# sid2364/dna-sequences-pg-extension

Hardware: NVIDIA B200
Metric: Gkmer/s counted (k=31) at 1/2/4/8 B200; extraction HBM GB/s vs peak (higher is better)
Workload: dtype u64

## Files before the change

dna-sequences-pg-extension_b200/csrc/dnagpu.cu:

```cuda
#include "../../include/dnagpu.h"

#include <cuda_runtime.h>

#include <algorithm>
#include <cmath>
#include <cstdarg>
#include <cstdio>
#include <cstdlib>
#include <cstring>
#include <new>
#include <string>
#include <thread>
#include <unordered_set>
#include <vector>

#include "kernels.cuh"
#include "partition.cuh"
#include "index.cuh"

using namespace dnagpu;

struct ProfRec {
    std::string name;
    cudaEvent_t e0, e1;
};

struct dnagpu_ctx {
    int device = 0;
    int sm_count = 0;
    cudaStream_t stream = nullptr;
    bool own_stream = true;
    unsigned long long *d_ctr = nullptr;
    int bins_ctas_per_sm = 4;
    unsigned long long *h_ctr = nullptr;
    cudaStream_t copy_stream = nullptr;
    std::vector<dnagpu_ctx *> peers;
    std::vector<uint64_t *> shard_buf;
    std::vector<uint64_t> shard_cap;
    bool profiling = false;
    bool plane_filter = false;
    bool force_exact = false;
    std::vector<ProfRec> prof;
    std::unordered_set<dnagpu_seq *> seqs;
    std::unordered_set<dnagpu_table *> tables;
    std::unordered_set<dnagpu_index *> indexes;
    char err[512] = {0};
};

struct dnagpu_seq {
    dnagpu_ctx *ctx = nullptr;
    int layout = kSingle;
    uint64_t *d_words = nullptr;
    bool own_words = true;
    uint64_t n_words_alloc = 0;
    uint64_t n_words = 0;
    uint64_t n_seqs = 1;
    uint64_t bases = 0;
    uint64_t stride = 0;
    uint64_t start_limit = 0;
    std::vector<uint64_t> h_n_bases;
    uint64_t *d_word_off = nullptr, *d_n_bases = nullptr;
    std::vector<const uint64_t *> piece_ptr;
    std::vector<uint64_t> piece_first, piece_starts;
    int cached_k = 0;
    uint64_t *d_row_off = nullptr, *d_item_off = nullptr;
    uint64_t cached_rows = 0, cached_items = 0;
};

struct dnagpu_table {
    dnagpu_ctx *ctx = nullptr;
    int k = 0;
    uint64_t rows = 0;
    uint64_t *d_kmers = nullptr, *d_counts = nullptr;
    std::vector<dnagpu_table *> parts;
};

struct dnagpu_index {
    dnagpu_ctx *ctx = nullptr;
    int k = 0;
    uint64_t rows = 0;
    uint64_t *d_skeys = nullptr, *d_rows = nullptr;
};

static thread_local char g_err[512] = "";

#ifdef DNAGPU_TUNING
// ... 160 lines not shown
    SMEM_ATTR(k_filter_collect<kSingle>);
    SMEM_ATTR(k_filter_collect<kFixed>);
    SMEM_ATTR(k_filter_collect<kRagged>);
    SMEM_ATTR((k_filter_sa<kSingle, kSaCollect>));
    SMEM_ATTR((k_filter_sa<kFixed, kSaCollect>));
    SMEM_ATTR((k_filter_sa<kSingle, kSaWrite>));
    SMEM_ATTR((k_filter_sa<kFixed, kSaWrite>));
    SMEM_ATTR((k_partition_write<kSingle, false>));
    SMEM_ATTR((k_partition_write<kSingle, true>));
    SMEM_ATTR((k_partition_write<kFixed, false>));
    SMEM_ATTR((k_partition_write<kFixed, true>));
    SMEM_ATTR((k_partition_write<kRagged, false>));
    SMEM_ATTR((k_partition_write<kRagged, true>));
    SMEM_ATTR((k_count_dense_smem<kSingle, false, uint32_t>));
    SMEM_ATTR((k_count_dense_smem<kSingle, true, uint32_t>));
    SMEM_ATTR((k_count_dense_smem<kFixed, false, uint32_t>));
    SMEM_ATTR((k_count_dense_smem<kFixed, true, uint32_t>));
    SMEM_ATTR((k_count_dense_smem<kRagged, false, uint32_t>));
    SMEM_ATTR((k_count_dense_smem<kRagged, true, uint32_t>));
    SMEM_ATTR((k_count_dense_smem<kSingle, false, unsigned long long>));
    SMEM_ATTR((k_count_dense_smem<kSingle, true, unsigned long long>));
    SMEM_ATTR((k_count_dense_smem<kFixed, false, unsigned long long>));
    SMEM_ATTR((k_count_dense_smem<kFixed, true, unsigned long long>));
    SMEM_ATTR((k_count_dense_smem<kRagged, false, unsigned long long>));
    SMEM_ATTR((k_count_dense_smem<kRagged, true, unsigned long long>));
#undef SMEM_ATTR
    {
        const int psmem = kTileKeys * (int)sizeof(uint64_t) + (int)sizeof(ScatterSmem);
#define PSMEM_ATTR(kern) cudaFuncSetAttribute(kern, cudaFuncAttributeMaxDynamicSharedMemorySize, psmem)
        PSMEM_ATTR((k_part_scatter_seq<kSingle, false>));
        PSMEM_ATTR((k_part_scatter_seq<kSingle, true>));
        PSMEM_ATTR((k_part_scatter_seq<kFixed, false>));
        PSMEM_ATTR((k_part_scatter_seq<kFixed, true>));
        PSMEM_ATTR((k_part_scatter_seq<kRagged, false>));
        PSMEM_ATTR((k_part_scatter_seq<kRagged, true>));
        PSMEM_ATTR(k_part_scatter_keys<false>);
        {
            const int psmem32 = 32 * kScatThreads * (int)sizeof(uint64_t) + (int)sizeof(ScatterSmem);
#define PSMEM32_ATTR(kern) cudaFuncSetAttribute(kern, cudaFuncAttributeMaxDynamicSharedMemorySize, psmem32)
            PSMEM32_ATTR((k_part_scatter_keys<false, kBigPerKeys, kBigThreadsKeys>));
            PSMEM32_ATTR((k_part_scatter_keys<true, kBigPerKeys, kBigThreadsKeys>));
            PSMEM32_ATTR((k_part_scatter_seq<kSingle, false, kBigPer, kBigThreads>));
            PSMEM32_ATTR((k_part_scatter_seq<kSingle, true, kBigPer, kBigThreads>));
            PSMEM32_ATTR((k_part_scatter_seq<kFixed, false, kBigPer, kBigThreads>));
            PSMEM32_ATTR((k_part_scatter_seq<kFixed, true, kBigPer, kBigThreads>));
            PSMEM32_ATTR((k_part_scatter_seq<kRagged, false, kBigPer, kBigThreads>));
            PSMEM32_ATTR((k_part_scatter_seq<kRagged, true, kBigPer, kBigThreads>));
#undef PSMEM32_ATTR
        }
        PSMEM_ATTR(k_part_scatter_keys<true>);
#undef PSMEM_ATTR
        {
            int per_sm = 0;
            if (cudaOccupancyMaxActiveBlocksPerMultiprocessor(&per_sm, k_count_buckets_bins, kThreads, 0) == cudaSuccess &&
                per_sm > 0)
                ctx->bins_ctas_per_sm = per_sm;
        }
        cudaFuncSetAttribute(k_sort_scatter<true>, cudaFuncAttributeMaxDynamicSharedMemorySize, (int)sizeof(SortSmem));
        cudaFuncSetAttribute(k_sort_scatter<false>, cudaFuncAttributeMaxDynamicSharedMemorySize, (int)sizeof(SortSmem));
        const int bsmem = kBucketSlots * 12;
        cudaFuncSetAttribute(k_count_buckets<false>, cudaFuncAttributeMaxDynamicSharedMemorySize, bsmem);
        cudaFuncSetAttribute(k_count_buckets<true>, cudaFuncAttributeMaxDynamicSharedMemorySize, bsmem);
    }
    CU(nullptr, cudaGetLastError());
    *out = ctx;
    return DNAGPU_OK;
}

extern "C" int dnagpu_create_multi(dnagpu_ctx **out, const int *devices, int n_devices)
{
    if (!out || !devices || n_devices < 1 || n_devices > kMaxPieces)
        return fail(nullptr, DNAGPU_EARG, "dnagpu_create_multi: need 1..%d devices", kMaxPieces);
    *out = nullptr;
    for (int a = 0; a < n_devices; ++a)
        for (int b = a + 1; b < n_devices; ++b)
            if (devices[a] == devices[b]) return fail(nullptr, DNAGPU_EARG, "device %d is listed twice", devices[a]);
    dnagpu_ctx *ctx = nullptr;
    TRY(dnagpu_create(&ctx, devices[0]));
    for (int d = 1; d < n_devices; ++d) {
        dnagpu_ctx *p = nullptr;
        int rc = dnagpu_create(&p, devices[d]);
        if (rc != DNAGPU_OK) {
            dnagpu_destroy(ctx);
            return rc;
        }
        ctx->peers.push_back(p);
    }
    for (int a = 0; a < n_devices; ++a) {
        cudaSetDevice(devices[a]);
        for (int b = 0; b < n_devices; ++b) {
            if (a == b) continue;
            int can = 0;
            cudaDeviceCanAccessPeer(&can, devices[a], devices[b]);
            cudaError_t e = can ? cudaDeviceEnablePeerAccess(devices[b], 0) : cudaErrorPeerAccessUnsupported;
            if (e == cudaErrorPeerAccessAlreadyEnabled) {
                cudaGetLastError();
                e = cudaSuccess;
            }
            if (e != cudaSuccess) {
                cudaGetLastError();
                dnagpu_destroy(ctx);
                return fail(nullptr, DNAGPU_ENODEVICE, "GPU %d cannot map the memory of GPU %d (%s): no multi-GPU context",
                            devices[a], devices[b], cudaGetErrorString(e));
            }
        }
    }
    cudaSetDevice(devices[0]);
    ctx->shard_buf.assign((size_t)n_devices, nullptr);
    ctx->shard_cap.assign((size_t)n_devices, 0);
// ... 1143 lines not shown
                k_part_hist_seq<LY, true><<<hgrid, kThreads, 0, ctx->stream>>>(in.v, in.p, mask, shift1, P1, hist1);
            else
                k_part_hist_seq<LY, false><<<hgrid, kThreads, 0, ctx->stream>>>(in.v, in.p, mask, shift1, P1, hist1);
        })));
    }
    TRY(scan_any(ctx, sc, (const uint64_t *)hist1, P1, off1));
    uint64_t *out = *keys_io;
    if (in.filtered || out)
        TRY(read_u64(ctx, off1 + P1, &n));
    if (!out) {
        TRY(sc.get((void **)&out, (n + 2) * 8));
        *keys_io = out;
    } else if (cap < n + 2) {
        *n_out = n;
        return fail(ctx, DNAGPU_ECAPACITY, "partition needs room for %llu keys (+2 pad)", (unsigned long long)n);
    }
    if (in.d_keys) {
        TRY(launch(ctx, "part_scatter", [&] {
            k_part_scatter_keys<true><<<grid_for(in.n, kTileKeys), kScatThreads, psmem, ctx->stream>>>(
                in.d_keys, root_off, root_off + 1, root_tiles_scat, 1, 1, shift1, P1, off1, cur1, out, ctx->d_ctr);
        }));
    } else {
        const bool per32 = scatter_tile32(P1, in.d_keys ? 0 : 1);
        if (per32) {
            const int psmem32 = 32 * kScatThreads * (int)sizeof(uint64_t) + (int)sizeof(ScatterSmem);
            const unsigned grid = grid_for(in.v.n_items, kScatThreads);
            DISPATCH_LAYOUT(in.seq->layout, TRY(launch(ctx, "part_scatter", [&] {
                if (in.filtered)
                    k_part_scatter_seq<LY, true, kBigPer, kBigThreads><<<grid, kBigThreads, psmem32, ctx->stream>>>(
                        in.v, in.p, mask, shift1, P1, off1, cur1, out, ctx->d_ctr, 0);
                else
                    k_part_scatter_seq<LY, false, kBigPer, kBigThreads><<<grid, kBigThreads, psmem32, ctx->stream>>>(
                        in.v, in.p, mask, shift1, P1, off1, cur1, out, ctx->d_ctr, 0);
            })));
        } else {
            const unsigned grid = grid_for(in.v.n_items, kScatThreads / 2);
            DISPATCH_LAYOUT(in.seq->layout, TRY(launch(ctx, "part_scatter", [&] {
                if (in.filtered)
                    k_part_scatter_seq<LY, true><<<grid, kScatThreads, psmem, ctx->stream>>>(
                        in.v, in.p, mask, shift1, P1, off1, cur1, out, ctx->d_ctr, 0);
                else
                    k_part_scatter_seq<LY, false><<<grid, kScatThreads, psmem, ctx->stream>>>(
                        in.v, in.p, mask, shift1, P1, off1, cur1, out, ctx->d_ctr, 0);
            })));
        }
    }
    *off1_out = off1;
    *n_out = n;
    return DNAGPU_OK;
}

static int part_finish_impl(dnagpu_ctx *ctx, Scratch &sc, const uint64_t *keys, uint64_t n, const uint64_t *parent_off,
                            const uint64_t *parent_end, uint64_t n_parents, uint64_t n_groups, int b1, int b2, int k,
                            dnagpu_stats *stats, uint64_t total_rows, dnagpu_table **table, bool optimistic2,
                            bool *regions_full)
{
    const int psmem = kTileKeys * (int)sizeof(uint64_t) + (int)sizeof(ScatterSmem);
    const uint64_t *bucket_keys = keys, *bucket_off = parent_off, *bucket_end = parent_end;
    uint64_t n_buckets = n_parents;
    *regions_full = false;
    if (b2 > 0) {
        const uint32_t P2 = 1u << b2;
        const int shift2 = 64 - b1 - b2;
        n_buckets = n_groups * P2;
        unsigned long long *hist2 = nullptr, *cur2;
        uint64_t *off2, *end2 = nullptr, *tiles_hist = nullptr, *tiles_scat, *bufB;
        TileInfo *tparent_hist = nullptr, *tparent_scat = nullptr;
        const uint64_t mean2 = (n + n_buckets - 1) / n_buckets;
        const uint64_t cap2 = mean2 + 7 * (uint64_t)std::ceil(std::sqrt((double)mean2)) + 64;
        TRY(sc.get((void **)&cur2, n_buckets * 8));
        TRY(sc.get((void **)&off2, (n_buckets + 1) * 8));
        CU(ctx, cudaMemsetAsync(cur2, 0, n_buckets * 8, ctx->stream));
        if (optimistic2) {
            TRY(sc.get((void **)&end2, n_buckets * 8));
            TRY(sc.get((void **)&bufB, (n_buckets * cap2 + 2) * 8));
            TRY(launch(ctx, "part_tiles", [&] {
                k_region_begs<<<grid_for(n_buckets, kThreads), kThreads, 0, ctx->stream>>>(cap2, n_buckets, off2);
            }));
        } else {
            TRY(sc.get((void **)&hist2, n_buckets * 8));
            TRY(sc.get((void **)&bufB, (n + 2) * 8));
            CU(ctx, cudaMemsetAsync(hist2, 0, n_buckets * 8, ctx->stream));
            TRY(part_tiles(ctx, sc, parent_off, parent_end, n_parents, kSuperTile, &tiles_hist, &tparent_hist,
                           (uint64_t)grid_for(n, kSuperTile) + n_parents));
        }
        const bool per32 = scatter_tile32(P2, 2);
        TRY(part_tiles(ctx, sc, parent_off, parent_end, n_parents, per32 ? 2 * kTileKeys : kTileKeys, &tiles_scat, &tparent_scat,
                       (uint64_t)grid_for(n, per32 ? 2 * kTileKeys : kTileKeys) + n_parents));
        if (!optimistic2) {
            TRY(launch(ctx, "part_hist2", [&] {
                k_part_hist_keys<<<grid_for(n, kSuperTile) + (unsigned)n_parents, kThreads, 0, ctx->stream>>>(
                    keys, parent_off, parent_end, tiles_hist, n_parents, n_groups, shift2, P2, hist2, tparent_hist);
            }));
            TRY(scan_any(ctx, sc, (const uint64_t *)hist2, n_buckets, off2));
        }
        const uint64_t cap = optimistic2 ? cap2 : 0;
        TRY(launch(ctx, "part_scatter2", [&] {
            if (per32) {
                const int psmem32 = 32 * kScatThreads * (int)sizeof(uint64_t) + (int)sizeof(ScatterSmem);
                k_part_scatter_keys<false, kBigPerKeys, kBigThreadsKeys><<<grid_for(n, 2 * kTileKeys) + (unsigned)n_parents, kBigThreadsKeys, psmem32,
                                                 ctx->stream>>>(keys, parent_off, parent_end, tiles_scat, n_parents, n_groups,
                                                                shift2, P2, off2, cur2, bufB, ctx->d_ctr, cap, C_L2OVF,
                                                                tparent_scat);
            } else {
                k_part_scatter_keys<false><<<grid_for(n, kTileKeys) + (unsigned)n_parents, kScatThreads, psmem, ctx->stream>>>(
                    keys, parent_off, parent_end, tiles_scat, n_parents, n_groups, shift2, P2, off2, cur2, bufB, ctx->d_ctr,
                    cap, C_L2OVF, tparent_scat);
            }
        }));
        bucket_keys = bufB;
        bucket_off = off2;
        bucket_end = off2 + 1;
        if (optimistic2) {
            TRY(launch(ctx, "part_tiles", [&] {
                k_region_ends<<<grid_for(n_buckets, kThreads), kThreads, 0, ctx->stream>>>(cur2, off2, cap2, (uint32_t)n_buckets,
                                                                                         end2);
            }));
            bucket_end = end2;
        }
    }
    const uint64_t spill_cap = std::max<uint64_t>(1ull << 16, n / 64);
    Slot *spill;
    TRY(sc.get((void **)&spill, spill_cap * sizeof(Slot)));
    TRY(launch(ctx, "table_init", [&] {
        k_table_init<<<(unsigned)std::min<uint64_t>(grid_for(spill_cap, kThreads), (uint64_t)ctx->sm_count * 8),
                       kThreads, 0, ctx->stream>>>(spill, spill_cap);
    }));
    const int bsmem = kBucketSlots * 12;
    const unsigned cgrid = (unsigned)std::min<uint64_t>(n_buckets, (uint64_t)ctx->sm_count * (16384 / kBucketSlots));
    static const bool use_bins = !tune_env("DNAGPU_NO_BINS");
    if (use_bins) {
        uint32_t *passed;
        TRY(sc.get((void **)&passed, n_buckets * 4 + 16));
        const unsigned bgrid = (unsigned)std::min<uint64_t>(n_buckets, (uint64_t)ctx->sm_count * ctx->bins_ctas_per_sm);
        TRY(launch(ctx, "count_buckets", [&] {
            k_count_buckets_bins<<<bgrid, kThreads, 0, ctx->stream>>>(bucket_keys, bucket_off, bucket_end, n_buckets,
                                                                     ctx->d_ctr, passed, ctx->d_ctr + C_PASSED);
        }));
        TRY(launch(ctx, "count_buckets_passed", [&] {
            k_count_buckets<false><<<cgrid, kThreads, bsmem, ctx->stream>>>(bucket_keys, bucket_off, bucket_end, n_buckets,
                                                                           spill, spill_cap, ctx->d_ctr, nullptr, nullptr,
                                                                           passed, ctx->d_ctr + C_PASSED);
        }));
    } else {
        TRY(launch(ctx, "count_buckets", [&] {
            k_count_buckets<false><<<cgrid, kThreads, bsmem, ctx->stream>>>(bucket_keys, bucket_off, bucket_end, n_buckets,
                                                                           spill, spill_cap, ctx->d_ctr, nullptr, nullptr);
        }));
    }
    TRY(fetch_counters(ctx));
    if (ctx->h_ctr[C_L2OVF]) {
        *regions_full = true;
        return DNAGPU_OK;
    }
#ifdef DNAGPU_PHASE_TIMING
    fprintf(stderr, "count_buckets phases (cycles/bucket, thread 0): init %.0f | sync %.0f | insert %.0f | prefetch+sync %.0f | buckets %llu\n",
            (double)ctx->h_ctr[110] / ctx->h_ctr[114], (double)ctx->h_ctr[111] / ctx->h_ctr[114],
            (double)ctx->h_ctr[112] / ctx->h_ctr[114], (double)ctx->h_ctr[113] / ctx->h_ctr[114],
            (unsigned long long)ctx->h_ctr[114]);
    fprintf(stderr, "scatter_seq phases (cycles/tile, thread 0): load+rank %.0f | barrier %.0f | plan %.0f | place %.0f+sync | flush %.0f | tiles %llu\n",
            (double)ctx->h_ctr[100] / ctx->h_ctr[105], (double)ctx->h_ctr[101] / ctx->h_ctr[105],
            (double)ctx->h_ctr[102] / ctx->h_ctr[105], (double)ctx->h_ctr[103] / ctx->h_ctr[105],
            (double)ctx->h_ctr[104] / ctx->h_ctr[105], (unsigned long long)ctx->h_ctr[105]);
#endif
    if (ctx->h_ctr[C_OVERFLOW])
        return fail(ctx, DNAGPU_EINTERNAL, "spill table of %llu slots overflowed", (unsigned long long)spill_cap);
    const uint64_t side = ctx->h_ctr[C_SIDE];
    const uint64_t keyed = ctx->h_ctr[C_DISTINCT];
    stats->total = total_rows ? total_rows : ctx->h_ctr[C_TOTAL];
    stats->distinct = keyed + (side > 0);
    stats->unique = ctx->h_ctr[C_UNIQUE] + (side == 1);
    if (table) {
        TRY(table_new(ctx, k, stats->distinct, table));
        if (keyed) {
            CU(ctx, cudaMemsetAsync(ctx->d_ctr + C_CURSOR, 0, 8, ctx->stream));
            TRY(launch(ctx, "count_buckets_emit", [&] {
                k_count_buckets<true><<<cgrid, kThreads, bsmem, ctx->stream>>>(
                    bucket_keys, bucket_off, bucket_end, n_buckets, spill, spill_cap, ctx->d_ctr, (*table)->d_kmers,
                    (*table)->d_counts);
            }));
            TRY(launch(ctx, "table_compact", [&] {
                k_table_compact<<<(unsigned)std::min<uint64_t>(grid_for(spill_cap, kThreads), (uint64_t)ctx->sm_count * 8),
                                  kThreads, 0, ctx->stream>>>(spill, spill_cap, (*table)->d_kmers,
                                                              (*table)->d_counts, ctx->d_ctr);
            }));
        }
        if (side) {
            ctx->h_ctr[0] = kEmpty;
            ctx->h_ctr[1] = side;
            CU(ctx, cudaMemcpyAsync((*table)->d_kmers + keyed, &ctx->h_ctr[0], 8, cudaMemcpyHostToDevice, ctx->stream));
            CU(ctx, cudaMemcpyAsync((*table)->d_counts + keyed, &ctx->h_ctr[1], 8, cudaMemcpyHostToDevice, ctx->stream));
        }
        CU(ctx, cudaStreamSynchronize(ctx->stream));
    }
    return DNAGPU_OK;
}

static int part_finish(dnagpu_ctx *ctx, Scratch &sc, const uint64_t *keys, uint64_t n, const uint64_t *parent_off,
                       const uint64_t *parent_end, uint64_t n_parents, uint64_t n_groups, int b1, int b2, int k,
                       dnagpu_stats *stats, uint64_t total_rows, dnagpu_table **table)
{
    static const bool allow = !tune_env("DNAGPU_EXACT_L2");
    const bool optimistic2 = allow && !ctx->force_exact && b2 > 0 && n_groups == n_parents && (n >> (b1 + b2)) >= 512;
    bool full = false;
    TRY(part_finish_impl(ctx, sc, keys, n, parent_off, parent_end, n_parents, n_groups, b1, b2, k, stats, total_rows, table,
                         optimistic2, &full));
    if (!full) return DNAGPU_OK;
    CU(ctx, cudaMemsetAsync(ctx->d_ctr + C_DISTINCT, 0, 2 * 8, ctx->stream));
    CU(ctx, cudaMemsetAsync(ctx->d_ctr + C_OVERFLOW, 0, 2 * 8, ctx->stream));
    CU(ctx, cudaMemsetAsync(ctx->d_ctr + C_L2OVF, 0, 2 * 8, ctx->stream));
    if (table && *table) {
        dnagpu_table_free(*table);
        *table = nullptr;
    }
    return part_finish_impl(ctx, sc, keys, n, parent_off, parent_end, n_parents, n_groups, b1, b2, k, stats, total_rows, table,
                            false, &full);
}

struct L1Regions {
    uint64_t *keys = nullptr, *beg = nullptr, *end = nullptr;
    unsigned long long *cur = nullptr;
    uint64_t cap = 0;
    uint32_t P1 = 0;
    int b1 = 0;
};

static int l1_regions_begin(dnagpu_ctx *ctx, Scratch &sc, uint64_t n_rows, int b1, L1Regions *r)
{
    r->b1 = b1;
    r->P1 = 1u << b1;
    const uint64_t mean = n_rows >> b1;
    r->cap = mean + mean / 8 + std::min<uint64_t>(65536, std::max<uint64_t>(1024, mean / 2));
    TRY(sc.get((void **)&r->keys, ((uint64_t)r->P1 * r->cap + 2) * 8));
    TRY(sc.get((void **)&r->beg, (uint64_t)r->P1 * 8));
    TRY(sc.get((void **)&r->end, (uint64_t)r->P1 * 8));
    TRY(sc.get((void **)&r->cur, (uint64_t)r->P1 * 8));
    TRY(launch(ctx, "part_tiles", [&] {
        k_region_begs<<<grid_for(r->P1, kThreads), kThreads, 0, ctx->stream>>>(r->cap, r->P1, r->beg);
    }));
    CU(ctx, cudaMemsetAsync(r->cur, 0, (uint64_t)r->P1 * 8, ctx->stream));
    return DNAGPU_OK;
}

static int l1_regions_scatter(dnagpu_ctx *ctx, const L1Regions &r, int layout, const SeqView &v, int k)
{
    const Pred none = {~0ull, ~0ull, ~0ull, ~0ull};
    if (scatter_tile32(r.P1, 1)) {
        const int psmem = 32 * kScatThreads * (int)sizeof(uint64_t) + (int)sizeof(ScatterSmem);
        const unsigned grid = grid_for(v.n_items, kScatThreads);
        DISPATCH_LAYOUT(layout, TRY(launch(ctx, "part_scatter", [&] {
            k_part_scatter_seq<LY, false, kBigPer, kBigThreads><<<grid, kBigThreads, psmem, ctx->stream>>>(
                v, none, kmer_mask(k), 64 - r.b1, r.P1, r.beg, r.cur, r.keys, ctx->d_ctr, r.cap);
        })));
        return DNAGPU_OK;
    }
    const int psmem = kTileKeys * (int)sizeof(uint64_t) + (int)sizeof(ScatterSmem);
    const unsigned grid = grid_for(v.n_items, kScatThreads / 2);
    DISPATCH_LAYOUT(layout, TRY(launch(ctx, "part_scatter", [&] {
        k_part_scatter_seq<LY, false><<<grid, kScatThreads, psmem, ctx->stream>>>(
            v, none, kmer_mask(k), 64 - r.b1, r.P1, r.beg, r.cur, r.keys, ctx->d_ctr, r.cap);
    })));
    return DNAGPU_OK;
}

static int l1_regions_scatter_keys(dnagpu_ctx *ctx, Scratch &sc, const L1Regions &r, const uint64_t *d_keys, uint64_t n)
{
    uint64_t *root_off, *tiles;
    TRY(sc.get((void **)&root_off, 2 * 8));
    ctx->h_ctr[C_COUNT] = 0;
    ctx->h_ctr[C_COUNT + 1] = n;
    CU(ctx, cudaMemcpyAsync(root_off, ctx->h_ctr + C_COUNT, 16, cudaMemcpyHostToDevice, ctx->stream));
    CU(ctx, cudaStreamSynchronize(ctx->stream));
    TRY(part_tiles(ctx, sc, root_off, root_off + 1, 1, 2 * kTileKeys, &tiles));
    const int psmem32 = 32 * kScatThreads * (int)sizeof(uint64_t) + (int)sizeof(ScatterSmem);
    return launch(ctx, "part_scatter", [&] {
        k_part_scatter_keys<true, kBigPerKeys, kBigThreadsKeys><<<grid_for(n, 2 * kTileKeys), kBigThreadsKeys, psmem32, ctx->stream>>>(
            d_keys, root_off, root_off + 1, tiles, 1, 1, 64 - r.b1, r.P1, r.beg, r.cur, r.keys, ctx->d_ctr, r.cap, C_L1OVF);
    });
}

static int l1_regions_end(dnagpu_ctx *ctx, const L1Regions &r)
{
    return launch(ctx, "part_tiles", [&] {
        k_region_ends<<<grid_for(r.P1, kThreads), kThreads, 0, ctx->stream>>>(r.cur, r.beg, r.cap, r.P1, r.end);
    });
}

static int count_partition_exact(dnagpu_ctx *ctx, const CountInput &in, int k, dnagpu_stats *stats,
                                 dnagpu_table **table)
{
    Scratch sc(ctx);
    int b1, b2;
    plan_bits(in.n, 1, &b1, &b2);
    TRY(zero_counters(ctx));
    uint64_t *off1, n, *keys = nullptr;
    TRY(part_level1(ctx, sc, in, k, b1, &keys, 0, &off1, &n));
    if (in.filtered) {
        int e1, e2;
        plan_bits(n, 1, &e1, &e2);
        b2 = std::max(0, std::min(11, e1 + e2 - b1));
    }
    const uint64_t P1 = 1ull << b1;
    return part_finish(ctx, sc, keys, n, off1, off1 + 1, P1, P1, b1, b2, k, stats, 0, table);
}

static int count_partition(dnagpu_ctx *ctx, const CountInput &in, int k, dnagpu_stats *stats,
                           dnagpu_table **table)
{
    static const bool no_optimistic = tune_env("DNAGPU_EXACT_LEVEL1") != nullptr;
    if (in.filtered || no_optimistic || ctx->force_exact || (in.d_keys && in.n < (1ull << 24)))
        return count_partition_exact(ctx, in, k, stats, table);
    {
        Scratch sc(ctx);
        int b1, b2;
        plan_bits(in.n, 1, &b1, &b2);
        TRY(zero_counters(ctx));
        L1Regions r;
        TRY(l1_regions_begin(ctx, sc, in.n, b1, &r));
        if (in.d_keys)
            TRY(l1_regions_scatter_keys(ctx, sc, r, in.d_keys, in.n));
        else
            TRY(l1_regions_scatter(ctx, r, in.seq->layout, in.v, k));
        TRY(l1_regions_end(ctx, r));
        TRY(part_finish(ctx, sc, r.keys, in.n, r.beg, r.end, r.P1, r.P1, b1, b2, k, stats, 0, table));
        if (!ctx->h_ctr[C_L1OVF]) return DNAGPU_OK;
        if (table && *table) {
            dnagpu_table_free(*table);
            *table = nullptr;
        }
    }
    return count_partition_exact(ctx, in, k, stats, table);
}

static int chunk_copy(dnagpu_ctx *ctx, std::vector<cudaEvent_t> &ev, uint64_t *dst, const uint64_t *src, uint64_t bytes)
{
    cudaEvent_t e;
    cudaError_t err = cudaEventCreateWithFlags(&e, cudaEventDisableTiming);
    if (err != cudaSuccess) return fail(ctx, DNAGPU_ECUDA, "cudaEventCreate: %s", cudaGetErrorString(err));
    ev.push_back(e);
    err = cudaMemcpyAsync(dst, src, bytes, cudaMemcpyHostToDevice, ctx->copy_stream);
    if (err == cudaSuccess) err = cudaEventRecord(e, ctx->copy_stream);
    if (err == cudaSuccess) err = cudaStreamWaitEvent(ctx->stream, e, 0);
    if (err != cudaSuccess) return fail(ctx, DNAGPU_ECUDA, "pipelined H2D copy: %s", cudaGetErrorString(err));
    return DNAGPU_OK;
}

static int count_kmers_pipelined(dnagpu_ctx *ctx, const uint64_t *words, uint64_t n_bases, int k,
                                 dnagpu_stats *stats, dnagpu_table **table, bool *done)
{
    *done = false;
    const uint64_t rows = rows_of(n_bases, k), n_words = words_of(n_bases);
    if (tune_env("DNAGPU_EXACT_LEVEL1") || pick_method(nullptr, k, rows) != DNAGPU_COUNT_PARTITION) return DNAGPU_OK;
    CU(ctx, cudaSetDevice(ctx->device));
    if (!ctx->copy_stream) CU(ctx, cudaStreamCreateWithFlags(&ctx->copy_stream, cudaStreamNonBlocking));
    Scratch sc(ctx);
    uint64_t *d_words;
    const uint64_t alloc_words = (n_words + 3) & ~1ull;
    TRY(sc.get((void **)&d_words, alloc_words * 8));
    CU(ctx, cudaMemsetAsync(d_words + n_words, 0, (alloc_words - n_words) * 8, ctx->stream));
    int b1, b2;
    plan_bits(rows, 1, &b1, &b2);
    TRY(zero_counters(ctx));
    L1Regions r;
    TRY(l1_regions_begin(ctx, sc, rows, b1, &r));
    CU(ctx, cudaStreamSynchronize(ctx->stream));
    const int n_chunks = 8;
    const uint64_t chunk_words = ((n_words + n_chunks - 1) / n_chunks + 255) & ~255ull;
    std::vector<cudaEvent_t> ev;
    int rc = DNAGPU_OK;
    for (uint64_t w0 = 0; w0 < n_words && rc == DNAGPU_OK; w0 += chunk_words) {
        const uint64_t w1 = std::min(n_words, w0 + chunk_words);
        const uint64_t copy_end = std::min(n_words, w1 + 1);
        rc = chunk_copy(ctx, ev, d_words + w0, words + w0, (copy_end - w0) * 8);
        if (rc != DNAGPU_OK) break;
        const uint64_t row0 = w0 * 32, row1 = std::min(rows, w1 * 32);
        if (row1 <= row0) continue;
        SeqView v;
        memset(&v, 0, sizeof v);
        v.words = d_words + w0;
        v.n_seqs = 1;
        v.rows_per_seq = v.n_rows = row1 - row0;
        v.items_per_seq = v.n_items = (v.n_rows + 31) / 32;
        rc = l1_regions_scatter(ctx, r, kSingle, v, k);
    }
    if (rc == DNAGPU_OK) rc = l1_regions_end(ctx, r);
    if (rc == DNAGPU_OK) rc = part_finish(ctx, sc, r.keys, rows, r.beg, r.end, r.P1, r.P1, b1, b2, k, stats, 0, table);
    cudaStreamSynchronize(ctx->copy_stream);
    if (rc != DNAGPU_OK) cudaStreamSynchronize(ctx->stream);
    for (cudaEvent_t e : ev) cudaEventDestroy(e);
    TRY(rc);
    if (ctx->h_ctr[C_L1OVF]) {
        if (table && *table) {
            dnagpu_table_free(*table);
            *table = nullptr;
        }
        dnagpu_seq *seq = nullptr;
        TRY(dnagpu_seq_wrap(ctx, d_words, n_bases, alloc_words, &seq));
        rc = dnagpu_count(ctx, seq, k, nullptr, nullptr, stats, table);
        dnagpu_seq_free(seq);
        TRY(rc);
    }
    *done = true;
    return DNAGPU_OK;
}

static int collect_launch(dnagpu_ctx *ctx, int layout, const SeqView &v, const Pred &p, int k, uint64_t *d_out, uint64_t cap)
{
    if (layout != kRagged && !ctx->plane_filter) {
        const SaPred sp = sa_pred_of(p, k);
        const uint64_t runs = layout == kSingle ? (v.n_items + kSaItems - 1) / kSaItems
                                                : v.n_seqs * ((v.items_per_seq + kSaItems - 1) / kSaItems);
        const int smem = kSaStage * (int)sizeof(uint64_t);
        return launch(ctx, "filter_collect", [&] {
            if (layout == kSingle)
                k_filter_sa<kSingle, kSaCollect><<<grid_for(runs, kThreads), kThreads, smem, ctx->stream>>>(
                    v, sp, kmer_mask(k), k, cap, ctx->d_ctr + C_CURSOR, nullptr, d_out);
            else
                k_filter_sa<kFixed, kSaCollect><<<grid_for(runs, kThreads), kThreads, smem, ctx->stream>>>(
                    v, sp, kmer_mask(k), k, cap, ctx->d_ctr + C_CURSOR, nullptr, d_out);
        });
    }
    const unsigned tiles = grid_for(v.n_items, kThreads);
    const int smem = kThreads * 32 * (int)sizeof(uint64_t);
    DISPATCH_LAYOUT(layout, TRY(launch(ctx, "filter_collect", [&] {
        k_filter_collect<LY><<<(tiles + kFilterTiles - 1) / kFilterTiles, kThreads, smem, ctx->stream>>>(
            v, p, kmer_mask(k), cap, ctx->d_ctr + C_CURSOR, d_out);
    })));
    return DNAGPU_OK;
}

static int collect_rows(dnagpu_ctx *ctx, const CountInput &in, int k, uint64_t *d_out, uint64_t cap, uint64_t *n_match)
{
    TRY(zero_counters(ctx));
    TRY(collect_launch(ctx, in.seq->layout, in.v, in.p, k, d_out, cap));
    return read_u64(ctx, (const uint64_t *)(ctx->d_ctr + C_CURSOR), n_match);
}

static int count_dense_any(dnagpu_ctx *ctx, const CountInput &in, int k, dnagpu_stats *stats, dnagpu_table **table);
static int count_partition(dnagpu_ctx *ctx, const CountInput &in, int k, dnagpu_stats *stats, dnagpu_table **table);
// ... 604 lines not shown
{
    if (!ctx || !seq || !plan || !d_out || !digit_counts)
        return fail(ctx, DNAGPU_EARG, "dnagpu_shuffle_send: NULL argument");
    TRY(check_k(ctx, k));
    TRY(check_filter_literals(ctx, filter));
    CU(ctx, cudaSetDevice(ctx->device));
    CountInput in;
    in.seq = seq;
    TRY(make_view(ctx, seq, k, &in.v));
    in.n = in.v.n_rows;
    TRY(build_pred(ctx, filter, k, in.n, &in.p, &in.filtered));
    for (uint32_t d = 0; d < plan->n_digits; ++d) digit_counts[d] = 0;
    if (rows_kept) *rows_kept = 0;
    if (side_rows) *side_rows = 0;
    if (in.n == 0) return DNAGPU_OK;
    Scratch sc(ctx);
    TRY(zero_counters(ctx));
    uint64_t *off1, n = 0, *keys = d_out;
    TRY(part_level1(ctx, sc, in, k, plan->bits1, &keys, cap, &off1, &n));
    std::vector<uint64_t> off((size_t)plan->n_digits + 1);
    CU(ctx, cudaMemcpyAsync(off.data(), off1, off.size() * 8, cudaMemcpyDeviceToHost, ctx->stream));
    TRY(fetch_counters(ctx));
    for (uint32_t d = 0; d < plan->n_digits; ++d) digit_counts[d] = off[d + 1] - off[d];
    if (rows_kept) *rows_kept = ctx->h_ctr[C_TOTAL];
    if (side_rows) *side_rows = ctx->h_ctr[C_SIDE];
    return DNAGPU_OK;
}

extern "C" int dnagpu_shuffle_count(dnagpu_ctx *ctx, const uint64_t *d_keys, const uint64_t *piece_counts,
                                    uint32_t n_pieces, uint32_t n_groups, const dnagpu_shuffle_plan *plan, int k,
                                    dnagpu_stats *stats, dnagpu_table **table)
{
    if (!ctx || !plan || !piece_counts || !stats || n_groups == 0 || n_pieces % n_groups)
        return fail(ctx, DNAGPU_EARG, "dnagpu_shuffle_count: bad arguments");
    TRY(check_k(ctx, k));
    CU(ctx, cudaSetDevice(ctx->device));
    stats->total = stats->distinct = stats->unique = 0;
    if (table) *table = nullptr;
    std::vector<uint64_t> off((size_t)n_pieces + 1, 0);
    for (uint32_t i = 0; i < n_pieces; ++i) off[i + 1] = off[i] + piece_counts[i];
    const uint64_t n = off[n_pieces];
    if (n == 0) {
        if (table) TRY(table_new(ctx, k, 0, table));
        return DNAGPU_OK;
    }
    if (!d_keys) return fail(ctx, DNAGPU_EARG, "dnagpu_shuffle_count: d_keys is NULL");
    Scratch sc(ctx);
    uint64_t *d_off;
    TRY(sc.get((void **)&d_off, off.size() * 8));
    CU(ctx, cudaMemcpyAsync(d_off, off.data(), off.size() * 8, cudaMemcpyHostToDevice, ctx->stream));
    CU(ctx, cudaStreamSynchronize(ctx->stream));
    TRY(zero_counters(ctx));
    int rc = part_finish(ctx, sc, d_keys, n, d_off, d_off + 1, n_pieces, n_groups, plan->bits1, plan->bits2, k, stats, n,
                         table);
    if (rc != DNAGPU_OK && table && *table) {
        dnagpu_table_free(*table);
        *table = nullptr;
    }
    return rc;
}

extern "C" int dnagpu_peer_alloc(dnagpu_ctx *ctx, uint64_t bytes, void **d_ptr, unsigned char handle[64])
{
    if (!ctx || !d_ptr || !handle) return fail(ctx, DNAGPU_EARG, "dnagpu_peer_alloc: NULL argument");
    static_assert(sizeof(cudaIpcMemHandle_t) == 64, "IPC handle size");
    CU(ctx, cudaSetDevice(ctx->device));
    *d_ptr = nullptr;
    cudaError_t e = cudaMalloc(d_ptr, bytes ? bytes : 16);
    if (e != cudaSuccess) {
        cudaGetLastError();
        return fail(ctx, DNAGPU_ENOMEM, "peer allocation of %llu bytes failed: %s", (unsigned long long)bytes,
                    cudaGetErrorString(e));
    }
    cudaIpcMemHandle_t h;
    e = cudaIpcGetMemHandle(&h, *d_ptr);
    if (e != cudaSuccess) {
        cudaFree(*d_ptr);
        *d_ptr = nullptr;
        cudaGetLastError();
        return fail(ctx, DNAGPU_ECUDA, "cudaIpcGetMemHandle: %s", cudaGetErrorString(e));
    }
    memcpy(handle, &h, 64);
    return DNAGPU_OK;
}

extern "C" int dnagpu_peer_open(dnagpu_ctx *ctx, const unsigned char handle[64], void **d_ptr)
{
    if (!ctx || !d_ptr || !handle) return fail(ctx, DNAGPU_EARG, "dnagpu_peer_open: NULL argument");
    CU(ctx, cudaSetDevice(ctx->device));
    cudaIpcMemHandle_t h;
    memcpy(&h, handle, 64);
    cudaError_t e = cudaIpcOpenMemHandle(d_ptr, h, cudaIpcMemLazyEnablePeerAccess);
    if (e != cudaSuccess) {
        cudaGetLastError();
        return fail(ctx, DNAGPU_ECUDA, "cudaIpcOpenMemHandle: %s (is peer access available between the GPUs?)",
                    cudaGetErrorString(e));
    }
    return DNAGPU_OK;
}

extern "C" int dnagpu_peer_close(dnagpu_ctx *ctx, void *d_ptr)
{
    if (!ctx) return fail(ctx, DNAGPU_EARG, "ctx is NULL");
    CU(ctx, cudaSetDevice(ctx->device));
    if (d_ptr) CU(ctx, cudaIpcCloseMemHandle(d_ptr));
    return DNAGPU_OK;
}
// ... 436 lines not shown
```

dna-sequences-pg-extension_b200/csrc/partition.cuh:

```cuda
#pragma once
#include "kernels.cuh"

namespace dnagpu {

constexpr int kScatThreads = 512;
constexpr int kScatPer = 16;
constexpr int kTileKeys = kScatThreads * kScatPer;
constexpr int kSuperTile = kTileKeys * 8;
constexpr int kMaxFan = 2048;
constexpr int kBigPer = 16, kBigThreads = 1024;
constexpr int kBigPerKeys = 32, kBigThreadsKeys = 512;
#ifndef DNAGPU_BUCKET_SLOTS
#define DNAGPU_BUCKET_SLOTS 4096
#endif
constexpr int kBucketSlots = DNAGPU_BUCKET_SLOTS;
constexpr int kBucketSlotBits = kBucketSlots == 4096 ? 12 : kBucketSlots == 8192 ? 13 : kBucketSlots == 2048 ? 11 : -1;
static_assert(kBucketSlotBits > 0, "DNAGPU_BUCKET_SLOTS must be 2048, 4096 or 8192");
constexpr uint64_t kSlotMul = 0x9E3779B97F4A7C15ull;
constexpr uint64_t kPartMul = 0xD6E8FEB86659FD93ull;

__device__ __forceinline__ uint64_t part_hash(uint64_t x) { return x * kPartMul; }
__device__ __forceinline__ uint32_t digit_of(uint64_t h, int shift, uint32_t fan_mask)
{
    return (uint32_t)(h >> shift) & fan_mask;
// ... 791 lines not shown
        }
        for (uint64_t i = beg + (uint64_t)kPre * kThreads + threadIdx.x; i < end; i += kThreads)
            bucket_insert(tk, tc, ld_nc(keys + i), !EMIT, spill, spill_cap, bt, ty, ctr);
        CT_MARK(c3);
#pragma unroll
        for (int u = 0; u < kPre; ++u) {
            uint64_t i = nbeg + (uint64_t)u * kThreads + threadIdx.x;
            pre[u] = i < nend ? ld_nc(keys + i) : kEmpty;
        }
        __syncthreads();
#ifdef DNAGPU_PHASE_TIMING
        {
            long long c4 = clock64();
            ph[0] += c1 - c0; ph[1] += c2 - c1; ph[2] += c3 - c2; ph[3] += c4 - c3; nbk++;
        }
#endif
        if (EMIT) {
            uint32_t mine = 0;
            for (int i = threadIdx.x; i < kBucketSlots; i += kThreads) mine += (tk[i] != kEmpty);
            uint32_t total;
            uint32_t rank = block_exscan(mine, &total);
            if (threadIdx.x == 0) row_base = atomicAdd(&ctr[C_CURSOR], (unsigned long long)total);
            __syncthreads();
            uint64_t pos = row_base + rank;
            for (int i = threadIdx.x; i < kBucketSlots; i += kThreads)
                if (tk[i] != kEmpty) {
                    out_kmers[pos] = tk[i];
                    out_counts[pos] = (uint64_t)tc[i] + 1;
                    pos++;
                }
            __syncthreads();
        }
        b = nb;
        beg = nbeg;
        end = nend;
    }
#ifdef DNAGPU_PHASE_TIMING
    if (threadIdx.x == 0) {
        for (int i = 0; i < 4; ++i) atomicAdd(&ctr[110 + i], (unsigned long long)ph[i]);
        atomicAdd(&ctr[114], (unsigned long long)nbk);
    }
#endif
    uint32_t d = warp_sum32(bt.distinct);
    int32_t u = (int32_t)__reduce_add_sync(0xffffffffu, bt.unique);
    if ((threadIdx.x & 31) == 0) {
        if (d) atomicAdd(&ctr[C_DISTINCT], (unsigned long long)d);
        if (u) atomicAdd(&ctr[C_UNIQUE], (unsigned long long)(long long)u);
    }
    ty.total = 0;
    tally_flush(ty, ctr);
}

constexpr int kBins = 2048;
constexpr int kBinPer = 12;
constexpr int kBinCap = kBinPer * kThreads;
constexpr int kBinWarpCap = kBinCap / (kThreads / 32);
constexpr int kBinHeavy = 15;
static_assert(kBins == 8 * kThreads && kBinCap <= 4096, "packing of k_count_buckets_bins");

__device__ __forceinline__ uint32_t bin_of(uint64_t x)
{
    return (((uint32_t)x ^ (uint32_t)(x >> 32)) * 0x9E3779B1u) >> 21;
}

template <int ROWS>
__device__ __forceinline__ void bins_rank(const uint64_t (&x)[kBinPer], uint32_t (&f)[kBinPer / 2], uint32_t n,
                                          uint32_t tid, uint32_t lane, uint32_t *cnt)
{
#pragma unroll
    for (int u = 0; u < ROWS; ++u) {
        const uint32_t bin = u * kThreads + tid < n ? bin_of(x[u]) : kBins + lane;
        const uint32_t v = bin | (atomicAdd(&cnt[bin], 1u) << 12);
        f[u >> 1] = (u & 1) ? __byte_perm(f[u >> 1], v, 0x5410) : v;
    }
}

template <int ROWS>
__device__ __forceinline__ void bins_load(uint64_t (&x)[kBinPer], const uint64_t *__restrict__ src, uint32_t n, uint32_t tid)
{
#pragma unroll
    for (int u = 0; u < ROWS; ++u)
        if (u * kThreads + tid < n) x[u] = ld_nc(src + u * kThreads);
}

template <int ROWS>
__device__ __forceinline__ void bins_place(const uint64_t (&x)[kBinPer], const uint32_t (&f)[kBinPer / 2],
                                           const uint16_t *st, uint64_t *stage, uint8_t *rank_at)
{
#pragma unroll
    for (int u = 0; u < ROWS; ++u) {
        const uint32_t v = (u & 1) ? (f[u >> 1] >> 16) : (f[u >> 1] & 0xffffu);
        const uint32_t pos = st[v & 0xfffu] + (v >> 12);
        stage[pos] = x[u];
        rank_at[pos] = (uint8_t)(v >> 12);
    }
}

#define BINS_DISPATCH(n, CALL)                                   \
    do {                                                         \
        if ((n) <= 4 * kThreads) { constexpr int ROWS = 4; CALL; } \
        else if ((n) <= 6 * kThreads) { constexpr int ROWS = 6; CALL; } \
        else if ((n) <= 8 * kThreads) { constexpr int ROWS = 8; CALL; } \
        else { constexpr int ROWS = kBinPer; CALL; }               \
    } while (0)

__global__ void __launch_bounds__(kThreads, 4) k_count_buckets_bins(const uint64_t *__restrict__ keys,
                                                                    const uint64_t *__restrict__ bucket_off,
                                                                    const uint64_t *__restrict__ bucket_end,
                                                                    uint64_t n_buckets,
                                                                    unsigned long long *__restrict__ ctr,
                                                                    uint32_t *__restrict__ list,
                                                                    unsigned long long *__restrict__ list_n)
{
    __shared__ __align__(16) uint64_t stage_raw[4 + kBinCap + 48];
    uint64_t *const stage = stage_raw + 4;
    __shared__ __align__(16) uint32_t cnt[kBins + 32];
    __shared__ __align__(16) uint16_t st[kBins + 32];
    __shared__ __align__(16) uint8_t rank_at[kBinCap + 48];
    const uint32_t tid = threadIdx.x, lane = tid & 31, warp = tid >> 5;
    uint32_t repeats = 0, second = 0;
    unsigned long long placed = 0;
    for (int i = tid; i < kBins + 32; i += kThreads) cnt[i] = 0;
    if (tid < 32) st[kBins + tid] = (uint16_t)(kBinCap + tid);
    uint64_t b = blockIdx.x;
    uint32_t n = 0;
    uint64_t x[kBinPer];
#pragma unroll
    for (int u = 0; u < kBinPer; ++u) x[u] = 0;
    if (b < n_buckets) {
        const uint64_t beg = bucket_off[b];
        n = (uint32_t)min(bucket_end[b] - beg, (uint64_t)kBinCap + 1);
        if (n <= kBinCap) BINS_DISPATCH(n, bins_load<ROWS>(x, keys + beg + tid, n, tid));
    }
    __syncthreads();
    while (b < n_buckets) {
        const uint64_t nb = b + gridDim.x;
        uint64_t nbeg = 0;
        uint32_t nn = 0;
        if (nb < n_buckets) {
            nbeg = bucket_off[nb];
            nn = (uint32_t)min(bucket_end[nb] - nbeg, (uint64_t)kBinCap + 1);
        }
        bool pass_on = n > kBinCap;
        uint32_t wtotal = 0;
        if (!pass_on) {
            uint32_t f[kBinPer / 2];
            BINS_DISPATCH(n, bins_rank<ROWS>(x, f, n, tid, lane, cnt));
            __syncthreads();
            const uint4 c0 = *reinterpret_cast<const uint4 *>(&cnt[8 * tid]);
            const uint4 c1 = *reinterpret_cast<const uint4 *>(&cnt[8 * tid + 4]);
            *reinterpret_cast<uint4 *>(&cnt[8 * tid]) = make_uint4(0, 0, 0, 0);
            *reinterpret_cast<uint4 *>(&cnt[8 * tid + 4]) = make_uint4(0, 0, 0, 0);
            const uint32_t s1 = c0.x, s2 = s1 + c0.y, s3 = s2 + c0.z, s4 = s3 + c0.w, s5 = s4 + c1.x, s6 = s5 + c1.y,
                           s7 = s6 + c1.z, mine = s7 + c1.w;
            const uint32_t worst = max(max(max(c0.x, c0.y), max(c0.z, c0.w)), max(max(c1.x, c1.y), max(c1.z, c1.w)));
            uint32_t inc = mine;
#pragma unroll
            for (int o = 1; o < 32; o <<= 1) {
                const uint32_t y = __shfl_up_sync(0xffffffffu, inc, o);
                if (lane >= o) inc += y;
            }
            wtotal = __shfl_sync(0xffffffffu, inc, 31);
            const bool bad = wtotal > (uint32_t)kBinWarpCap || worst > (uint32_t)kBinHeavy;
            const uint32_t p = warp * kBinWarpCap + inc - mine;
            *reinterpret_cast<uint4 *>(&st[8 * tid]) =
                make_uint4(p | ((p + s1) << 16), (p + s2) | ((p + s3) << 16), (p + s4) | ((p + s5) << 16),
                           (p + s6) | ((p + s7) << 16));
            pass_on = __syncthreads_or(bad);
            if (!pass_on) {
                BINS_DISPATCH(n, bins_place<ROWS>(x, f, st, stage, rank_at));
                if (tid == 0) placed += n;
            }
        }
        if (nn <= kBinCap) BINS_DISPATCH(nn, bins_load<ROWS>(x, keys + nbeg + tid, nn, tid));
        if (n <= kBinCap) {
            __syncthreads();
            if (!pass_on) {
                const uint32_t base = warp * kBinWarpCap;
                for (uint32_t q = base + lane; q < base + wtotal; q += 32) {
                    const uint32_t r = rank_at[q];
                    const uint64_t key = stage[q], k1 = stage[q - 1], k2 = stage[q - 2], k3 = stage[q - 3];
                    uint32_t e = (uint32_t)((r >= 1) & (k1 == key)) + (uint32_t)((r >= 2) & (k2 == key)) +
                                 (uint32_t)((r >= 3) & (k3 == key));
                    if (r > 3) {
#pragma unroll 1
                        for (uint32_t j = 4; j <= r; ++j) e += stage[q - j] == key;
                    }
                    repeats += e >= 1;
                    second += e == 1;
                }
            }
        }
        if (pass_on && tid == 0) list[atomicAdd(list_n, 1ull)] = (uint32_t)b;
        b = nb;
        n = nn;
    }
    repeats = warp_sum32(repeats);
    second = warp_sum32(second);
    if (lane == 0 && (repeats | second)) {
        atomicAdd(&ctr[C_DISTINCT], (unsigned long long)(-(long long)repeats));
        atomicAdd(&ctr[C_UNIQUE], (unsigned long long)(-(long long)repeats - (long long)second));
    }
    if (tid == 0 && placed) {
        atomicAdd(&ctr[C_DISTINCT], placed);
        atomicAdd(&ctr[C_UNIQUE], placed);
    }
}

constexpr int kScanPer = 8;
__global__ void __launch_bounds__(1024) k_scan_block(const uint64_t *__restrict__ in, uint64_t n,
                                                     uint64_t *__restrict__ out,
                                                     uint64_t *__restrict__ block_sums)
{
    __shared__ uint64_t wtot[32];
    const int lane = threadIdx.x & 31, wid = threadIdx.x >> 5;
    const uint64_t base = ((uint64_t)blockIdx.x * 1024 + threadIdx.x) * kScanPer;
    uint64_t v[kScanPer], sum = 0;
#pragma unroll
    for (int i = 0; i < kScanPer; ++i) {
        v[i] = base + i < n ? in[base + i] : 0;
        sum += v[i];
    }
    uint64_t inc = sum;
#pragma unroll
    for (int o = 1; o < 32; o <<= 1) {
        uint64_t y = __shfl_up_sync(0xffffffffu, inc, o);
        if (lane >= o) inc += y;
    }
    if (lane == 31) wtot[wid] = inc;
    __syncthreads();
    if (wid == 0) {
        uint64_t t = wtot[lane], ti = t;
#pragma unroll
        for (int o = 1; o < 32; o <<= 1) {
// ... 28 lines not shown
```

Before: 66.95.

## Stage 32-bit hashed residues in bins counting kernel when partition bits are shared

```diff
diff --git a/dna-sequences-pg-extension_b200/csrc/dnagpu.cu b/dna-sequences-pg-extension_b200/csrc/dnagpu.cu
--- a/dna-sequences-pg-extension_b200/csrc/dnagpu.cu
+++ b/dna-sequences-pg-extension_b200/csrc/dnagpu.cu
@@ -31,7 +31,7 @@
     cudaStream_t stream = nullptr;
     bool own_stream = true;
     unsigned long long *d_ctr = nullptr;
-    int bins_ctas_per_sm = 4;
+    int bins_ctas_per_sm[2] = {4, 4};
     unsigned long long *h_ctr = nullptr;
     cudaStream_t copy_stream = nullptr;
     std::vector<dnagpu_ctx *> peers;
@@ -298,9 +298,13 @@
 #undef PSMEM_ATTR
         {
             int per_sm = 0;
-            if (cudaOccupancyMaxActiveBlocksPerMultiprocessor(&per_sm, k_count_buckets_bins, kThreads, 0) == cudaSuccess &&
+            if (cudaOccupancyMaxActiveBlocksPerMultiprocessor(&per_sm, k_count_buckets_bins<uint64_t>, kThreads, 0) == cudaSuccess &&
                 per_sm > 0)
-                ctx->bins_ctas_per_sm = per_sm;
+                ctx->bins_ctas_per_sm[0] = per_sm;
+            per_sm = 0;
+            if (cudaOccupancyMaxActiveBlocksPerMultiprocessor(&per_sm, k_count_buckets_bins<uint32_t>, kThreads, 0) == cudaSuccess &&
+                per_sm > 0)
+                ctx->bins_ctas_per_sm[1] = per_sm;
         }
         cudaFuncSetAttribute(k_sort_scatter<true>, cudaFuncAttributeMaxDynamicSharedMemorySize, (int)sizeof(SortSmem));
         cudaFuncSetAttribute(k_sort_scatter<false>, cudaFuncAttributeMaxDynamicSharedMemorySize, (int)sizeof(SortSmem));
@@ -1550,8 +1554,8 @@
 
 static int part_finish_impl(dnagpu_ctx *ctx, Scratch &sc, const uint64_t *keys, uint64_t n, const uint64_t *parent_off,
                             const uint64_t *parent_end, uint64_t n_parents, uint64_t n_groups, int b1, int b2, int k,
-                            dnagpu_stats *stats, uint64_t total_rows, dnagpu_table **table, bool optimistic2,
-                            bool *regions_full)
+                            int shared_bits, dnagpu_stats *stats, uint64_t total_rows, dnagpu_table **table,
+                            bool optimistic2, bool *regions_full)
 {
     const int psmem = kTileKeys * (int)sizeof(uint64_t) + (int)sizeof(ScatterSmem);
     const uint64_t *bucket_keys = keys, *bucket_off = parent_off, *bucket_end = parent_end;
@@ -1630,10 +1634,17 @@
     if (use_bins) {
         uint32_t *passed;
         TRY(sc.get((void **)&passed, n_buckets * 4 + 16));
-        const unsigned bgrid = (unsigned)std::min<uint64_t>(n_buckets, (uint64_t)ctx->sm_count * ctx->bins_ctas_per_sm);
+        const int bin_shift = 64 - shared_bits - kBinBits;
+        const bool residue = shared_bits > 0 && bin_shift <= 32;
+        const unsigned bgrid =
+            (unsigned)std::min<uint64_t>(n_buckets, (uint64_t)ctx->sm_count * ctx->bins_ctas_per_sm[residue ? 1 : 0]);
         TRY(launch(ctx, "count_buckets", [&] {
-            k_count_buckets_bins<<<bgrid, kThreads, 0, ctx->stream>>>(bucket_keys, bucket_off, bucket_end, n_buckets,
-                                                                     ctx->d_ctr, passed, ctx->d_ctr + C_PASSED);
+            if (residue)
+                k_count_buckets_bins<uint32_t><<<bgrid, kThreads, 0, ctx->stream>>>(
+                    bucket_keys, bucket_off, bucket_end, n_buckets, ctx->d_ctr, passed, ctx->d_ctr + C_PASSED, bin_shift);
+            else
+                k_count_buckets_bins<uint64_t><<<bgrid, kThreads, 0, ctx->stream>>>(
+                    bucket_keys, bucket_off, bucket_end, n_buckets, ctx->d_ctr, passed, ctx->d_ctr + C_PASSED, 0);
         }));
         TRY(launch(ctx, "count_buckets_passed", [&] {
             k_count_buckets<false><<<cgrid, kThreads, bsmem, ctx->stream>>>(bucket_keys, bucket_off, bucket_end, n_buckets,
@@ -1696,13 +1707,13 @@
 
 static int part_finish(dnagpu_ctx *ctx, Scratch &sc, const uint64_t *keys, uint64_t n, const uint64_t *parent_off,
                        const uint64_t *parent_end, uint64_t n_parents, uint64_t n_groups, int b1, int b2, int k,
-                       dnagpu_stats *stats, uint64_t total_rows, dnagpu_table **table)
+                       dnagpu_stats *stats, uint64_t total_rows, dnagpu_table **table, int shared_bits = 0)
 {
     static const bool allow = !tune_env("DNAGPU_EXACT_L2");
     const bool optimistic2 = allow && !ctx->force_exact && b2 > 0 && n_groups == n_parents && (n >> (b1 + b2)) >= 512;
     bool full = false;
-    TRY(part_finish_impl(ctx, sc, keys, n, parent_off, parent_end, n_parents, n_groups, b1, b2, k, stats, total_rows, table,
-                         optimistic2, &full));
+    TRY(part_finish_impl(ctx, sc, keys, n, parent_off, parent_end, n_parents, n_groups, b1, b2, k, shared_bits, stats,
+                         total_rows, table, optimistic2, &full));
     if (!full) return DNAGPU_OK;
     CU(ctx, cudaMemsetAsync(ctx->d_ctr + C_DISTINCT, 0, 2 * 8, ctx->stream));
     CU(ctx, cudaMemsetAsync(ctx->d_ctr + C_OVERFLOW, 0, 2 * 8, ctx->stream));
@@ -1711,8 +1722,8 @@
         dnagpu_table_free(*table);
         *table = nullptr;
     }
-    return part_finish_impl(ctx, sc, keys, n, parent_off, parent_end, n_parents, n_groups, b1, b2, k, stats, total_rows, table,
-                            false, &full);
+    return part_finish_impl(ctx, sc, keys, n, parent_off, parent_end, n_parents, n_groups, b1, b2, k, shared_bits, stats,
+                            total_rows, table, false, &full);
 }
 
 struct L1Regions {
@@ -1799,7 +1810,7 @@
         b2 = std::max(0, std::min(11, e1 + e2 - b1));
     }
     const uint64_t P1 = 1ull << b1;
-    return part_finish(ctx, sc, keys, n, off1, off1 + 1, P1, P1, b1, b2, k, stats, 0, table);
+    return part_finish(ctx, sc, keys, n, off1, off1 + 1, P1, P1, b1, b2, k, stats, 0, table, b1 + b2);
 }
 
 static int count_partition(dnagpu_ctx *ctx, const CountInput &in, int k, dnagpu_stats *stats,
@@ -1820,7 +1831,7 @@
         else
             TRY(l1_regions_scatter(ctx, r, in.seq->layout, in.v, k));
         TRY(l1_regions_end(ctx, r));
-        TRY(part_finish(ctx, sc, r.keys, in.n, r.beg, r.end, r.P1, r.P1, b1, b2, k, stats, 0, table));
+        TRY(part_finish(ctx, sc, r.keys, in.n, r.beg, r.end, r.P1, r.P1, b1, b2, k, stats, 0, table, b1 + b2));
         if (!ctx->h_ctr[C_L1OVF]) return DNAGPU_OK;
         if (table && *table) {
             dnagpu_table_free(*table);
@@ -1882,7 +1893,7 @@
         rc = l1_regions_scatter(ctx, r, kSingle, v, k);
     }
     if (rc == DNAGPU_OK) rc = l1_regions_end(ctx, r);
-    if (rc == DNAGPU_OK) rc = part_finish(ctx, sc, r.keys, rows, r.beg, r.end, r.P1, r.P1, b1, b2, k, stats, 0, table);
+    if (rc == DNAGPU_OK) rc = part_finish(ctx, sc, r.keys, rows, r.beg, r.end, r.P1, r.P1, b1, b2, k, stats, 0, table, b1 + b2);
     cudaStreamSynchronize(ctx->copy_stream);
     if (rc != DNAGPU_OK) cudaStreamSynchronize(ctx->stream);
     for (cudaEvent_t e : ev) cudaEventDestroy(e);
@@ -2593,7 +2604,7 @@
     CU(ctx, cudaStreamSynchronize(ctx->stream));
     TRY(zero_counters(ctx));
     int rc = part_finish(ctx, sc, d_keys, n, d_off, d_off + 1, n_pieces, n_groups, plan->bits1, plan->bits2, k, stats, n,
-                         table);
+                         table, 0);
     if (rc != DNAGPU_OK && table && *table) {
         dnagpu_table_free(*table);
         *table = nullptr;
diff --git a/dna-sequences-pg-extension_b200/csrc/partition.cuh b/dna-sequences-pg-extension_b200/csrc/partition.cuh
--- a/dna-sequences-pg-extension_b200/csrc/partition.cuh
+++ b/dna-sequences-pg-extension_b200/csrc/partition.cuh
@@ -867,24 +867,29 @@
 }
 
 constexpr int kBins = 2048;
+constexpr int kBinBits = 11;
 constexpr int kBinPer = 12;
 constexpr int kBinCap = kBinPer * kThreads;
 constexpr int kBinWarpCap = kBinCap / (kThreads / 32);
 constexpr int kBinHeavy = 15;
 static_assert(kBins == 8 * kThreads && kBinCap <= 4096, "packing of k_count_buckets_bins");
+static_assert(kBins == 1 << kBinBits, "kBinBits");
 
 __device__ __forceinline__ uint32_t bin_of(uint64_t x)
 {
     return (((uint32_t)x ^ (uint32_t)(x >> 32)) * 0x9E3779B1u) >> 21;
 }
 
-template <int ROWS>
-__device__ __forceinline__ void bins_rank(const uint64_t (&x)[kBinPer], uint32_t (&f)[kBinPer / 2], uint32_t n,
-                                          uint32_t tid, uint32_t lane, uint32_t *cnt)
+template <typename T, int ROWS>
+__device__ __forceinline__ void bins_rank(uint64_t (&x)[kBinPer], uint32_t (&f)[kBinPer / 2], uint32_t n,
+                                          uint32_t tid, uint32_t lane, uint32_t *cnt, int bin_shift)
 {
 #pragma unroll
     for (int u = 0; u < ROWS; ++u) {
-        const uint32_t bin = u * kThreads + tid < n ? bin_of(x[u]) : kBins + lane;
+        if (sizeof(T) != sizeof(uint64_t)) x[u] = part_hash(x[u]);
+        const uint32_t bin = u * kThreads + tid < n ? (sizeof(T) == sizeof(uint64_t) ? bin_of(x[u])
+                                                                                      : (uint32_t)(x[u] >> bin_shift) & (kBins - 1))
+                                                    : kBins + lane;
         const uint32_t v = bin | (atomicAdd(&cnt[bin], 1u) << 12);
         f[u >> 1] = (u & 1) ? __byte_perm(f[u >> 1], v, 0x5410) : v;
     }
@@ -898,15 +903,15 @@
         if (u * kThreads + tid < n) x[u] = ld_nc(src + u * kThreads);
 }
 
-template <int ROWS>
+template <typename T, int ROWS>
 __device__ __forceinline__ void bins_place(const uint64_t (&x)[kBinPer], const uint32_t (&f)[kBinPer / 2],
-                                           const uint16_t *st, uint64_t *stage, uint8_t *rank_at)
+                                           const uint16_t *st, T *stage, uint8_t *rank_at)
 {
 #pragma unroll
     for (int u = 0; u < ROWS; ++u) {
         const uint32_t v = (u & 1) ? (f[u >> 1] >> 16) : (f[u >> 1] & 0xffffu);
         const uint32_t pos = st[v & 0xfffu] + (v >> 12);
-        stage[pos] = x[u];
+        stage[pos] = (T)x[u];
         rank_at[pos] = (uint8_t)(v >> 12);
     }
 }
@@ -919,16 +924,18 @@
         else { constexpr int ROWS = kBinPer; CALL; }               \
     } while (0)
 
+template <typename T>
 __global__ void __launch_bounds__(kThreads, 4) k_count_buckets_bins(const uint64_t *__restrict__ keys,
                                                                     const uint64_t *__restrict__ bucket_off,
                                                                     const uint64_t *__restrict__ bucket_end,
                                                                     uint64_t n_buckets,
                                                                     unsigned long long *__restrict__ ctr,
                                                                     uint32_t *__restrict__ list,
-                                                                    unsigned long long *__restrict__ list_n)
-{
-    __shared__ __align__(16) uint64_t stage_raw[4 + kBinCap + 48];
-    uint64_t *const stage = stage_raw + 4;
+                                                                    unsigned long long *__restrict__ list_n,
+                                                                    int bin_shift)
+{
+    __shared__ __align__(16) T stage_raw[4 + kBinCap + 48];
+    T *const stage = stage_raw + 4;
     __shared__ __align__(16) uint32_t cnt[kBins + 32];
     __shared__ __align__(16) uint16_t st[kBins + 32];
     __shared__ __align__(16) uint8_t rank_at[kBinCap + 48];
@@ -960,7 +967,7 @@
         uint32_t wtotal = 0;
         if (!pass_on) {
             uint32_t f[kBinPer / 2];
-            BINS_DISPATCH(n, bins_rank<ROWS>(x, f, n, tid, lane, cnt));
+            BINS_DISPATCH(n, (bins_rank<T, ROWS>(x, f, n, tid, lane, cnt, bin_shift)));
             __syncthreads();
             const uint4 c0 = *reinterpret_cast<const uint4 *>(&cnt[8 * tid]);
             const uint4 c1 = *reinterpret_cast<const uint4 *>(&cnt[8 * tid + 4]);
@@ -983,7 +990,7 @@
                            (p + s6) | ((p + s7) << 16));
             pass_on = __syncthreads_or(bad);
             if (!pass_on) {
-                BINS_DISPATCH(n, bins_place<ROWS>(x, f, st, stage, rank_at));
+                BINS_DISPATCH(n, (bins_place<T, ROWS>(x, f, st, stage, rank_at)));
                 if (tid == 0) placed += n;
             }
         }
@@ -994,7 +1001,7 @@
                 const uint32_t base = warp * kBinWarpCap;
                 for (uint32_t q = base + lane; q < base + wtotal; q += 32) {
                     const uint32_t r = rank_at[q];
-                    const uint64_t key = stage[q], k1 = stage[q - 1], k2 = stage[q - 2], k3 = stage[q - 3];
+                    const T key = stage[q], k1 = stage[q - 1], k2 = stage[q - 2], k3 = stage[q - 3];
                     uint32_t e = (uint32_t)((r >= 1) & (k1 == key)) + (uint32_t)((r >= 2) & (k2 == key)) +
                                  (uint32_t)((r >= 3) & (k3 == key));
                     if (r > 3) {
```

Measured after the change: 69.15 (median of 6 runs). 1.03x the previous value.
